# vghuy17ck1/svt-av1-psyex

Measured on AMD Instinct MI355X. Metric: ME+RD-cost Mpixels/s (2160p10 preset-6), higher is better.
Workload: dtype u8 SAD / i32 transforms; 1 GPU; 3840x2160 10-bit synthetic pan sequence, preset 6 (M6) search controls at qp 35; step = 16 pictures (4 current pictures x ref distance 1,2,4,8; R=2): open-loop ME of all 2040 b64 + full-pel pred + RD chain (64x64,32x32,16x16 DCT_DCT, 10-bit, b quantizer; qcoeff + recon + scalars written); 3 picture sets alternate from step to step

## Files before the change

svt-av1-psyex_amd/csrc/rd_kernel.hip:

```cpp
#include <hip/hip_runtime.h>
#include <math.h>
#include <stdint.h>
#include <string.h>
#include <type_traits>
#include "svt_hip_internal.h"
#include "../../include/svt_hip_dsp.h"

#include "txfm_core.h"

namespace {

struct RdParams {
    SvtHipRdBatchDesc d;
    const int16_t    *iscan[3];
    int               tx_size;
};

template <typename T> __device__ __forceinline__ int ldpix(const void *p, size_t i) { return (int)static_cast<const T *>(p)[i]; }

__host__ __device__ constexpr int rd_lanes_per_block(int ts) { return tx_wide(ts) > tx_high(ts) ? tx_wide(ts) : tx_high(ts); }
__host__ __device__ constexpr int rd_blocks_per_wave(int ts) { return 64 / rd_lanes_per_block(ts); }

#ifndef SVT_RD_WAVES_64
#define SVT_RD_WAVES_64 2
#endif
#ifndef SVT_RD_WAVES_32
#define SVT_RD_WAVES_32 4
#endif
#ifndef SVT_RD_RESIDUAL_AHEAD
#define SVT_RD_RESIDUAL_AHEAD 8
#endif
#ifndef SVT_RD_SCAN_AHEAD
#define SVT_RD_SCAN_AHEAD 16
#endif
#ifndef SVT_RD_WAVES_16
#define SVT_RD_WAVES_16 4
#endif
__host__ __device__ constexpr int rd_waves_per_simd(int ts) {
    return rd_lanes_per_block(ts) == 64 ? SVT_RD_WAVES_64 : rd_lanes_per_block(ts) == 32 ? SVT_RD_WAVES_32 : SVT_RD_WAVES_16;
}
template <int TS, int BD> __global__ void __launch_bounds__(64, rd_waves_per_simd(TS)) rd_tx_kernel(const RdParams p) {
    constexpr int W = tx_wide(TS), H = tx_high(TS), WP = W > 32 ? 32 : W, HP = H > 32 ? 32 : H, NP = WP * HP;
    constexpr int LW = rd_lanes_per_block(TS), BPW = rd_blocks_per_wave(TS);
    constexpr bool kShift32 = LW != 32;
    constexpr int PA = W + 1, PB = WP + 1;
    constexpr int ROW_CLAMP = BD == 8 ? 16 : 18, COL_CLAMP = 16;
    constexpr bool RECT = (W == 2 * H || H == 2 * W);
    using Pix = typename std::conditional<BD == 8, uint8_t, uint16_t>::type;
    __shared__ int32_t lds[BPW][H * PA];
    const int      lane = threadIdx.x, blk = lane / LW, l = lane % LW;
    const uint32_t job   = blockIdx.x * BPW + blk;
    const bool     valid = job < p.d.n_jobs;
    int32_t *A = lds[blk];
    const SvtHipTxJob jb = p.d.jobs[valid ? job : 0];
    const int tt = jb.tx_type & 15, vt = c_vtx[tt], ht = c_htx[tt];
    const bool ud = (vt == 2), lr = (ht == 2);
    const Pix *src  = static_cast<const Pix *>(p.d.src) + jb.src_offset;
    const Pix *pred = static_cast<const Pix *>(p.d.pred) + jb.pred_offset;
    const int8_t *fsh = c_fwd_shift[TS];
    const int bit_col = c_fwd_cos_col[ilog2c(W) - 2][ilog2c(H) - 2], bit_row = c_fwd_cos_row[ilog2c(W) - 2][ilog2c(H) - 2];

    constexpr int RUN = W < 8 ? W : 8, RPR = W / RUN;
    typedef Pix __attribute__((ext_vector_type(RUN), aligned(sizeof(Pix)))) RunU;
    uint32_t rmax = 0;
    {
        HiLo rhl;
        constexpr int NIT = (RPR * H + LW - 1) / LW, kResidualAhead = NIT < SVT_RD_RESIDUAL_AHEAD ? NIT : SVT_RD_RESIDUAL_AHEAD;
        for (int it0 = 0; it0 < NIT; it0 += kResidualAhead) {
            RunU sv[kResidualAhead], pv[kResidualAhead];
#pragma unroll
            for (int j = 0; j < kResidualAhead; j++) {
                const int i = l + (it0 + j) * LW;
                if (it0 + j < NIT && i < RPR * H) {
                    const int r = i / RPR, c = (i - r * RPR) * RUN;
                    sv[j] = *reinterpret_cast<const RunU *>(src + (size_t)r * p.d.src_stride + c);
                    pv[j] = *reinterpret_cast<const RunU *>(pred + (size_t)r * p.d.pred_stride + c);
                }
            }
#pragma unroll
            for (int j = 0; j < kResidualAhead; j++) {
                const int i = l + (it0 + j) * LW;
                if (it0 + j < NIT && i < RPR * H) {
                    const int r = i / RPR, c = (i - r * RPR) * RUN;
#pragma unroll
                    for (int k = 0; k < RUN; k++) {
                        const int32_t d = (int16_t)((int16_t)sv[j][k] - (int16_t)pv[j][k]);
                        A[r * PA + c + k] = d;
                        rhl.take(d);
                    }
                }
            }
        }
        rmax = rhl.max_abs();
    }
    const bool fast_col = pass_fits_17_bits((uint32_t)__builtin_amdgcn_readfirstlane((int)wave_max(rmax)) << (fsh[0] > 0 ? fsh[0] : 0), H);
    __syncthreads();
    uint32_t cmax = 0;
    if (l < W) {
        int32_t x[H];
#pragma unroll
        for (int r = 0; r < H; r++) x[r] = A[(ud ? H - 1 - r : r) * PA + l];
        shift_vec<H>(x, fsh[0]);
        if (fast_col) { fwd_1d<H, 2>(x, vt, bit_col); shift_vec<H, kShift32>(x, fsh[1]); } else { fwd_1d<H, 0>(x, vt, bit_col); shift_vec<H>(x, fsh[1]); }
        const int oc = lr ? W - 1 - l : l;
#pragma unroll
        for (int r = 0; r < H; r++) A[r * PA + oc] = x[r];
        cmax = vec_max_abs<H>(x);
    }
    const bool fast_row = pass_fits_17_bits((uint32_t)__builtin_amdgcn_readfirstlane((int)wave_max(cmax)), W);
    __syncthreads();
    uint32_t comax = 0;
    if (l < H) {
        int32_t x[W];
#pragma unroll
        for (int c = 0; c < W; c++) x[c] = A[l * PA + c];
        if (fast_row) { fwd_1d<W, 2>(x, ht, bit_row); shift_vec<W, kShift32>(x, fsh[2]); } else { fwd_1d<W, 0>(x, ht, bit_row); shift_vec<W>(x, fsh[2]); }
        if constexpr (RECT) {
#pragma unroll
            for (int c = 0; c < W; c++) x[c] = rshift64((i64)x[c] * 5793, 12);
        }
#pragma unroll
        for (int c = 0; c < W; c++) A[l * PA + c] = x[c];
        comax = vec_max_abs<W>(x);
    }
    const uint32_t comax_w = (uint32_t)__builtin_amdgcn_readfirstlane((int)wave_max(comax));
    const bool q24 = comax_w < (1u << 16);
    __syncthreads();
    const int pf = jb.pf_shape & 3;
    const int keep_w = pf == 3 ? 1 : (W >> pf), keep_h = pf == 3 ? 1 : (H >> pf);
    u64 tq = 0;
    if (pf == 0) if constexpr (W > 32 || H > 32) {
        for (int i = l; i < W * H; i += LW) {
            const int r = i / W, c = i - r * W;
            if (r >= HP || c >= WP) { const int32_t v = A[r * PA + c]; tq += (u64)((i64)v * v); }
        }
        tq = group_sum<LW>(tq);
    }
    if constexpr (W > 32 || H > 32) __syncthreads();
    const SvtHipQuantRow q = p.d.quant_rows[jb.quant_row];
    const int     log_scale = p.d.quant_kind == 2 ? 0 : c_log_scale[TS];
    const int16_t *iscan    = p.iscan[(tt >= 10) ? ((tt & 1) ? 2 : 1) : 0];
    const uint8_t *qm = (tt < 9) ? p.d.qmatrix : nullptr, *iqm = (tt < 9) ? p.d.iqmatrix : nullptr;
    uint32_t satd = 0, eob = 0, qsum = 0;
    int32_t  dc_q = 0;
    u64      dres = 0, dpred = 0;
    int32_t *co_out = (p.d.coeff && valid) ? p.d.coeff + (size_t)job * NP : nullptr;
    int32_t *q_out  = (p.d.qcoeff && valid) ? p.d.qcoeff + (size_t)job * NP : nullptr;
    int32_t *dq_out = (p.d.dqcoeff && valid) ? p.d.dqcoeff + (size_t)job * NP : nullptr;
    const int32_t zb_c[2]  = {log_scale ? ((q.zbin[0] + (1 << (log_scale - 1))) >> log_scale) : q.zbin[0], log_scale ? ((q.zbin[1] + (1 << (log_scale - 1))) >> log_scale) : q.zbin[1]};
    const int32_t rnd_c[2] = {log_scale ? ((q.round[0] + (1 << (log_scale - 1))) >> log_scale) : q.round[0], log_scale ? ((q.round[1] + (1 << (log_scale - 1))) >> log_scale) : q.round[1]};
    const bool fast_q = q24 && !qm && p.d.quant_kind == 0 && !co_out && !dq_out && __all(pf == 0);
    constexpr int LS = tx_log_scale(TS), KT = LS == 2 ? 4 : 3;
    bool lane_lean = fast_q && q_out != nullptr && log_scale == LS;
    {
        const int32_t  rndm = rnd_c[0] > rnd_c[1] ? rnd_c[0] : rnd_c[1], sm = q.quant_shift[0] > q.quant_shift[1] ? q.quant_shift[0] : q.quant_shift[1];
        const int32_t  dm = q.dequant[0] > q.dequant[1] ? q.dequant[0] : q.dequant[1], qm2 = (q.quant[0] > q.quant[1] ? q.quant[0] : q.quant[1]) + 65536;
        const bool     nonneg = (rnd_c[0] | rnd_c[1] | q.quant_shift[0] | q.quant_shift[1] | q.dequant[0] | q.dequant[1]) >= 0;
        uint32_t       tmax = comax_w + (uint32_t)(nonneg ? rndm : 0);
        if (BD == 8) tmax = tmax > 32767u ? 32767u : tmax;
        const u64 qvmax = ((((u64)tmax * (uint32_t)qm2) >> 11) * (u64)(uint32_t)(nonneg ? sm : 0)) >> (21 - LS);
        const u64 dqmax = (qvmax * (u64)(uint32_t)(nonneg ? dm : 0)) >> LS;
        const u64 M = dqmax > comax_w ? dqmax : (u64)comax_w;
        lane_lean = lane_lean && nonneg && tmax < (1u << (18 - KT)) && M < (1u << 16) && M * M * (NP / LW) < (1ull << 32);
    }
    const bool lean_q = __all(lane_lean);
    if (lean_q) {
        static_assert(NP % LW == 0, "every lane of a block walks the same number of coefficients");
        constexpr int kScanAhead = NP / LW < SVT_RD_SCAN_AHEAD ? ((NP / LW) & ~1) : SVT_RD_SCAN_AHEAD;
        static_assert(kScanAhead >= 2 && kScanAhead % 2 == 0 && NP / LW >= kScanAhead, "ahead of the loop");
// ... 137 lines not shown
                qv = (int32_t)(((((t * q.quant[ac]) >> 16) + t) * q.quant_shift[ac]) >> (16 - log_scale + 5));
                const int32_t deq = ((int32_t)q.dequant[ac] * iwt + 16) >> 5;
                dq = (qv * deq) >> log_scale;
            }
        } else if (!qm) {
            const bool keep = (BD == 8) ? (((i64)a << (1 + log_scale)) >= (int32_t)q.dequant[ac]) : ((a << (1 + log_scale)) >= q.dequant[ac]);
            if (keep) {
                i64 t = (i64)a + (log_scale ? ((q.round_fp[ac] + (1 << (log_scale - 1))) >> log_scale) : q.round_fp[ac]);
                if (BD == 8) t = t < -32768 ? -32768 : (t > 32767 ? 32767 : t);
                qv = (int32_t)((t * q.quant_fp[ac]) >> (16 - log_scale));
                dq = (qv * (int32_t)q.dequant[ac]) >> log_scale;
            }
        } else {
            if ((i64)a * wt >= ((int32_t)q.dequant[ac] << (5 - (1 + log_scale)))) {
                i64 t = (i64)a + (log_scale ? ((q.round_fp[ac] + (1 << (log_scale - 1))) >> log_scale) : q.round_fp[ac]);
                if (BD == 8) t = t < -32768 ? -32768 : (t > 32767 ? 32767 : t);
                qv = (int32_t)((t * q.quant_fp[ac] * wt) >> (16 - log_scale + 5));
                const int32_t deq = ((int32_t)q.dequant[ac] * iwt + 16) >> 5;
                dq = (qv * deq) >> log_scale;
            }
        }
        const int32_t qs = (qv ^ sign) - sign, dqs = (dq ^ sign) - sign;
        if (qv) { const uint32_t e = (uint32_t)iscan[rc] + 1; eob = e > eob ? e : eob; }
        qsum += (uint32_t)(qv > 63 ? 63 : qv);
        if (rc == 0) dc_q = qs;
        const i64 dd = (i64)co - dqs;
        dres += (u64)(dd * dd);
        dpred += (u64)((i64)co * co);
        A[r * PB + c] = dqs;
        if (co_out) co_out[rc] = co;
        if (q_out) q_out[rc] = qs;
        if (dq_out) dq_out[rc] = dqs;
    }
    satd  = group_sum<LW>(satd);
    qsum  = group_sum<LW>(qsum);
    eob   = group_max<LW>(eob);
    dres  = group_sum<LW>(dres);
    dpred = group_sum<LW>(dpred);
    __syncthreads();
    int32_t xr[W];
    uint32_t irmax = 0;
    if (l < H) {
#pragma unroll
        for (int c = 0; c < W; c++) {
            int32_t v = (l < HP && c < WP) ? A[l * PB + c] : 0;
            if constexpr (RECT) v = rshift64((i64)v * 2896, 12);
            xr[c] = clampv(v, BD + 8);
        }
        irmax = vec_max_abs<W>(xr);
    }
    const bool fast_irow = ipass_fits_18_bits((uint32_t)__builtin_amdgcn_readfirstlane((int)wave_max(irmax)), W);
    uint32_t icmax = 0;
    if (l < H) {
        if (fast_irow) inv_1d<W, ROW_CLAMP, 2>(xr, ht); else inv_1d<W, ROW_CLAMP, 1>(xr, ht);
        shift_vec<W, kShift32>(xr, c_inv_shift0[TS]);
#pragma unroll
        for (int c = 0; c < W; c++) A[l * PA + c] = xr[c];
        icmax = vec_max_abs<W>(xr);
    }
    const bool fast_icol = ipass_fits_18_bits((uint32_t)__builtin_amdgcn_readfirstlane((int)wave_max(icmax)), H);
    __syncthreads();
    u64 sse = 0;
    if (l < W) {
        int32_t x[H];
        const int ic = lr ? W - 1 - l : l;
#pragma unroll
        for (int r = 0; r < H; r++) x[r] = (r < HP) ? clampv(A[r * PA + ic], BD + 6 > 16 ? BD + 6 : 16) : 0;
        if (fast_icol) inv_1d<H, COL_CLAMP, 2>(x, vt); else inv_1d<H, COL_CLAMP, 1>(x, vt);
        shift_vec<H, kShift32>(x, -4);
#pragma unroll
        for (int r = 0; r < H; r++) A[r * PA + l] = x[ud ? H - 1 - r : r];
    }
    __syncthreads();
    {
        Pix *rec = (p.d.recon && valid) ? static_cast<Pix *>(p.d.recon) + jb.pred_offset : nullptr;
        constexpr int NIT = (RPR * H + LW - 1) / LW;
        RunU pv[NIT], sv[NIT];
#pragma unroll
        for (int it = 0; it < NIT; it++) {
            const int i = l + it * LW;
            if (i < RPR * H) {
                const int r = i / RPR, c = (i - r * RPR) * RUN;
                pv[it] = *reinterpret_cast<const RunU *>(pred + (size_t)r * p.d.pred_stride + c);
                sv[it] = *reinterpret_cast<const RunU *>(src + (size_t)r * p.d.src_stride + c);
            }
        }
#pragma unroll
        for (int it = 0; it < NIT; it++) {
            const int i = l + it * LW;
            if (i < RPR * H) {
                const int r = i / RPR, c = (i - r * RPR) * RUN;
                RunU out;
#pragma unroll
                for (int k = 0; k < RUN; k++) {
                    int v = (int)pv[it][k] + A[r * PA + c + k];
                    v = v < 0 ? 0 : (v > (1 << BD) - 1 ? (1 << BD) - 1 : v);
                    out[k] = (Pix)v;
                    const int e = (int)sv[it][k] - v;
                    sse += (u64)((uint32_t)e * (uint32_t)e);
                }
                if (rec) *reinterpret_cast<RunU *>(rec + (size_t)r * p.d.pred_stride + c) = out;
            }
        }
    }
    sse = group_sum<LW>(sse);
    if (l == 0 && valid) {
        p.d.eob[job]  = (uint16_t)eob;
        p.d.satd[job] = satd;
        p.d.dist_coeff[2 * (size_t)job]     = dres;
        p.d.dist_coeff[2 * (size_t)job + 1] = dpred;
        p.d.three_quad_energy[job] = tq;
        p.d.sse[job]  = sse;
        if (p.d.cul_level) p.d.cul_level[job] = (uint8_t)((qsum > 63 ? 63 : qsum) | (dc_q < 0 ? 64 : 0)) + (uint8_t)(dc_q > 0 ? 128 : 0);
    }
}

struct InvParams {
    SvtHipInvTxBatchDesc d;
};
template <int TS, int BD, typename Pix> __global__ void __launch_bounds__(64, rd_waves_per_simd(TS)) inv_tx_kernel(const InvParams p) {
    constexpr int W = tx_wide(TS), H = tx_high(TS), WP = W > 32 ? 32 : W, HP = H > 32 ? 32 : H, NP = WP * HP;
    constexpr int LW = rd_lanes_per_block(TS), BPW = rd_blocks_per_wave(TS);
    constexpr bool kShift32 = LW != 32;
    constexpr int PA = W + 1, PB = WP + 1;
    constexpr int ROW_CLAMP = BD == 8 ? 16 : 18, COL_CLAMP = 16;
    constexpr bool RECT = (W == 2 * H || H == 2 * W);
    __shared__ int32_t lds[BPW][H * PA];
    const int      lane = threadIdx.x, blk = lane / LW, l = lane % LW;
    const uint32_t job   = blockIdx.x * BPW + blk;
    const bool     valid = job < p.d.n_jobs;
    int32_t *A = lds[blk];
    const SvtHipTxJob jb = p.d.jobs[valid ? job : 0];
    const int tt = jb.tx_type & 15, vt = c_vtx[tt], ht = c_htx[tt];
    const bool ud = (vt == 2), lr = (ht == 2);
    const Pix *pred = static_cast<const Pix *>(p.d.pred) + jb.pred_offset;
    const int32_t *dq = p.d.dqcoeff + (size_t)(valid ? job : 0) * NP;
    for (int rc = l; rc < NP; rc += LW) { const int r = rc / WP, c = rc - r * WP; A[r * PB + c] = dq[rc]; }
    __syncthreads();
    int32_t xr[W];
    uint32_t irmax = 0;
    if (l < H) {
#pragma unroll
        for (int c = 0; c < W; c++) {
            int32_t v = (l < HP && c < WP) ? A[l * PB + c] : 0;
            if constexpr (RECT) v = rshift64((i64)v * 2896, 12);
            xr[c] = clampv(v, BD + 8);
        }
        irmax = vec_max_abs<W>(xr);
    }
    const bool fast_irow = ipass_fits_18_bits((uint32_t)__builtin_amdgcn_readfirstlane((int)wave_max(irmax)), W);
    uint32_t icmax = 0;
    if (l < H) {
        if (fast_irow) inv_1d<W, ROW_CLAMP, 2>(xr, ht); else inv_1d<W, ROW_CLAMP, 1>(xr, ht);
        shift_vec<W, kShift32>(xr, c_inv_shift0[TS]);
#pragma unroll
        for (int c = 0; c < W; c++) A[l * PA + c] = xr[c];
        icmax = vec_max_abs<W>(xr);
    }
    const bool fast_icol = ipass_fits_18_bits((uint32_t)__builtin_amdgcn_readfirstlane((int)wave_max(icmax)), H);
    __syncthreads();
    if (l < W) {
        int32_t x[H];
        const int ic = lr ? W - 1 - l : l;
#pragma unroll
        for (int r = 0; r < H; r++) x[r] = (r < HP) ? clampv(A[r * PA + ic], BD + 6 > 16 ? BD + 6 : 16) : 0;
        if (fast_icol) inv_1d<H, COL_CLAMP, 2>(x, vt); else inv_1d<H, COL_CLAMP, 1>(x, vt);
        shift_vec<H, kShift32>(x, -4);
#pragma unroll
        for (int r = 0; r < H; r++) A[r * PA + l] = x[ud ? H - 1 - r : r];
    }
    __syncthreads();
    if (valid) {
        Pix *rec = static_cast<Pix *>(p.d.recon) + jb.src_offset;
        for (int i = l; i < W * H; i += LW) {
            const int r = i / W, c = i - r * W;
            int v = (int)pred[(size_t)r * p.d.pred_stride + c] + A[r * PA + c];
            v = v < 0 ? 0 : (v > (1 << BD) - 1 ? (1 << BD) - 1 : v);
            rec[(size_t)r * p.d.recon_stride + c] = (Pix)v;
        }
    }
}

template <int BD, typename Pix> int launch_inv(SvtHipContext *ctx, const InvParams &p) {
    const dim3 b(64);
#define CASE(S) case S: hipLaunchKernelGGL((inv_tx_kernel<S, BD, Pix>), dim3((p.d.n_jobs + rd_blocks_per_wave(S) - 1) / rd_blocks_per_wave(S)), b, 0, ctx->stream, p); break;
    switch (p.d.tx_size) {
        CASE(0) CASE(1) CASE(2) CASE(3) CASE(4) CASE(5) CASE(6) CASE(7) CASE(8) CASE(9) CASE(10) CASE(11) CASE(12) CASE(13) CASE(14) CASE(15) CASE(16) CASE(17) CASE(18)
    default: return svt_hip_fail(ctx, SVT_HIP_ERR_BAD_PARAM, "tx_size %d", p.d.tx_size);
    }
#undef CASE
    SVT_HIP_CHECK(ctx, hipGetLastError());
    return SVT_HIP_OK;
}

struct FwdParams {
    SvtHipFwdTxBatchDesc d;
};
template <int TS> __global__ void __launch_bounds__(64, rd_waves_per_simd(TS)) fwd_tx_kernel(const FwdParams p) {
    constexpr int W = tx_wide(TS), H = tx_high(TS);
    constexpr int LW = rd_lanes_per_block(TS), BPW = rd_blocks_per_wave(TS);
    constexpr int PA = W + 1;
    constexpr bool RECT = (W == 2 * H || H == 2 * W);
    __shared__ int32_t lds[BPW][H * PA];
    const int      lane = threadIdx.x, blk = lane / LW, l = lane % LW;
    const uint32_t job   = blockIdx.x * BPW + blk;
    const bool     valid = job < p.d.n_jobs;
    int32_t *A = lds[blk];
    const SvtHipTxJob jb = p.d.jobs[valid ? job : 0];
    const int tt = jb.tx_type & 15, vt = c_vtx[tt], ht = c_htx[tt];
    const bool ud = (vt == 2), lr = (ht == 2);
    const int16_t *res = p.d.residual + jb.src_offset;
    const int8_t *fsh = c_fwd_shift[TS];
    const int bit_col = c_fwd_cos_col[ilog2c(W) - 2][ilog2c(H) - 2], bit_row = c_fwd_cos_row[ilog2c(W) - 2][ilog2c(H) - 2];
    uint32_t rmax = 0;
    for (int i = l; i < W * H; i += LW) {
        const int r = i / W, c = i - r * W;
        const int32_t d = res[(size_t)r * p.d.residual_stride + c];
        A[r * PA + c] = d;
        rmax = max(rmax, (uint32_t)(d < 0 ? -d : d));
    }
// ... 251 lines not shown
```

svt-av1-psyex_amd/csrc/txfm_core.h:

```cpp
#ifndef SVT_HIP_TXFM_CORE_H
#define SVT_HIP_TXFM_CORE_H
#include <hip/hip_runtime.h>
#include <math.h>
#include <stdint.h>
#include "wave_ops.h"

namespace {

typedef unsigned long long u64;
typedef long long          i64;

__constant__ int32_t c_cospi[4][64];
inline hipError_t txfm_upload_cospi() {
    int32_t cosp[4][64];
    for (int b = 0; b < 4; b++)
        for (int j = 0; j < 64; j++) cosp[b][j] = (int32_t)(cos(3.14159265358979323846 * j / 128.0) * (double)(1 << (10 + b)) + 0.5);
    return hipMemcpyToSymbol(HIP_SYMBOL(c_cospi), cosp, sizeof(cosp));
}
__constant__ int32_t c_sinpi[4][5] = {{0, 330, 621, 836, 951}, {0, 660, 1241, 1672, 1901}, {0, 1321, 2482, 3344, 3803}, {0, 2642, 4964, 6689, 7606}};

struct TxGeom { uint8_t w, h; };
__host__ __device__ constexpr int tx_wide(int s) { constexpr uint8_t t[19] = {4, 8, 16, 32, 64, 4, 8, 8, 16, 16, 32, 32, 64, 4, 16, 8, 32, 16, 64}; return t[s]; }
__host__ __device__ constexpr int tx_high(int s) { constexpr uint8_t t[19] = {4, 8, 16, 32, 64, 8, 4, 16, 8, 32, 16, 64, 32, 16, 4, 32, 8, 64, 16}; return t[s]; }
__host__ __device__ constexpr int ilog2c(int n) { return n <= 1 ? 0 : 1 + ilog2c(n >> 1); }
__host__ __device__ constexpr int brevc(int v, int bits) { int r = 0; for (int i = 0; i < bits; i++) r |= ((v >> i) & 1) << (bits - 1 - i); return r; }

__device__ const int8_t  c_fwd_shift[19][3] = {{2, 0, 0},  {2, -1, 0}, {2, -2, 0}, {2, -4, 0}, {0, -2, -2}, {2, -1, 0}, {2, -1, 0}, {2, -2, 0}, {2, -2, 0}, {2, -4, 0},
                                               {2, -4, 0}, {0, -2, -2}, {2, -4, -2}, {2, -1, 0}, {2, -1, 0}, {2, -2, 0}, {2, -2, 0}, {0, -2, 0}, {2, -4, 0}};
__device__ const int8_t  c_fwd_cos_col[5][5] = {{13, 13, 13, 0, 0}, {13, 13, 13, 12, 0}, {13, 13, 13, 12, 13}, {0, 13, 13, 12, 13}, {0, 0, 13, 12, 13}};
__device__ const int8_t  c_fwd_cos_row[5][5] = {{13, 13, 12, 0, 0}, {13, 13, 13, 12, 0}, {13, 13, 12, 13, 12}, {0, 12, 13, 12, 11}, {0, 0, 12, 11, 10}};
__device__ const int8_t  c_inv_shift0[19]    = {0, -1, -2, -2, -2, 0, 0, -1, -1, -1, -1, -1, -1, -1, -1, -2, -2, -2, -2};
__device__ const uint8_t c_log_scale[19]     = {0, 0, 0, 1, 2, 0, 0, 0, 0, 1, 1, 2, 2, 0, 0, 0, 0, 1, 1};
__device__ const uint8_t c_vtx[16] = {0, 1, 0, 1, 2, 0, 2, 1, 2, 3, 0, 3, 1, 3, 2, 3};
__device__ const uint8_t c_htx[16] = {0, 0, 1, 1, 0, 2, 2, 2, 1, 3, 3, 0, 3, 1, 3, 2};

__device__ __forceinline__ int32_t mul24_shr(int32_t a, int32_t b, int sh) {
    int32_t hi;
    asm("v_mul_hi_i32_i24 %0, %1, %2" : "=v"(hi) : "v"(a), "v"(b));
    return (int32_t)__builtin_amdgcn_alignbit((uint32_t)hi, (uint32_t)__mul24(a, b), (uint32_t)sh);
}
__device__ __forceinline__ uint32_t umul24_lo(uint32_t a, uint32_t b) {
    uint32_t lo;
    asm("v_mul_u32_u24 %0, %1, %2" : "=v"(lo) : "v"(a), "v"(b));
    return lo;
}
__device__ __forceinline__ uint32_t umul24_hi(uint32_t a, uint32_t b) {
    uint32_t hi;
    asm("v_mul_hi_u32_u24 %0, %1, %2" : "=v"(hi) : "v"(a), "v"(b));
    return hi;
}
__host__ __device__ constexpr int tx_log_scale(int s) { return tx_wide(s) * tx_high(s) > 1024 ? 2 : tx_wide(s) * tx_high(s) > 256 ? 1 : 0; }
__device__ __forceinline__ int32_t rshift64(i64 v, int bit) { return (int32_t)((v + ((i64)1 << (bit - 1))) >> bit); }
template <int MUL> __device__ __forceinline__ int32_t hbtf(int32_t w0, int32_t a, int32_t w1, int32_t b, int bit) {
    if constexpr (MUL == 2) return (__mul24(w1, b) + (__mul24(w0, a) + (1 << (bit - 1)))) >> bit;
    i64 s;
    if constexpr (MUL == 1) s = (i64)__mul24(w0, a) + (i64)__mul24(w1, b);
    else s = (i64)(int32_t)((uint32_t)w0 * (uint32_t)a) + (i64)(int32_t)((uint32_t)w1 * (uint32_t)b);
    return (int32_t)((s + ((i64)1 << (bit - 1))) >> bit);
}
__device__ __forceinline__ int32_t clamp32(int32_t v, int bit) {
    const int32_t hi = (1 << (bit - 1)) - 1, lo = -(1 << (bit - 1));
    return v < lo ? lo : (v > hi ? hi : v);
}
__device__ __forceinline__ int32_t clampv(i64 v, int bit) {
    const i64 hi = ((i64)1 << (bit - 1)) - 1, lo = -((i64)1 << (bit - 1));
    return (int32_t)(v < lo ? lo : (v > hi ? hi : v));
}
__device__ __forceinline__ int32_t clampv(int32_t v, int bit) { return clamp32(v, bit); }
__device__ __forceinline__ int32_t wadd(int32_t a, int32_t b) { return (int32_t)((uint32_t)a + (uint32_t)b); }
__device__ __forceinline__ int32_t wsub(int32_t a, int32_t b) { return (int32_t)((uint32_t)a - (uint32_t)b); }

template <int M, int K, int MUL> __device__ __forceinline__ void odd_rot(int32_t *x, const int32_t *c, int bit) {
    constexpr int t = M >> K;
    if constexpr (K == 1) {
#pragma unroll
        for (int j = 0; j < M / 4; j++) {
            const int p = M + M / 4 + j, m = 3 * M - 1 - p;
            const int32_t a = x[p], b = x[m];
            x[p] = hbtf<MUL>(-c[32], a, c[32], b, bit);
            x[m] = hbtf<MUL>(c[32], b, c[32], a, bit);
        }
    } else {
#pragma unroll
        for (int g = 0; g < (1 << (K - 2)); g++) {
            const int A = (1 + 4 * brevc(g, K - 2)) * (64 >> K), B = 64 - A, base = M + g * 2 * t;
#pragma unroll
            for (int j = 0; j < t / 2; j++) {
                const int p = base + t / 2 + j, m = 3 * M - 1 - p;
                const int32_t a = x[p], b = x[m];
                x[p] = hbtf<MUL>(-c[A], a, c[B], b, bit);
                x[m] = hbtf<MUL>(c[A], b, c[B], a, bit);
            }
#pragma unroll
            for (int j = 0; j < t / 2; j++) {
                const int p = base + t + j, m = 3 * M - 1 - p;
                const int32_t a = x[p], b = x[m];
                x[p] = hbtf<MUL>(-c[B], a, -c[A], b, bit);
                x[m] = hbtf<MUL>(c[B], b, -c[A], a, bit);
            }
        }
    }
}
template <int M, int K, int CLAMP> __device__ __forceinline__ void odd_bfly(int32_t *x) {
    constexpr int t = M >> K;
#pragma unroll
    for (int g = 0; g < M / t; g++) {
#pragma unroll
        for (int j = 0; j < t / 2; j++) {
            const int i0 = M + g * t + j, i1 = M + g * t + t - 1 - j;
            const int32_t lo = x[i0], hi = x[i1];
            int32_t s, d;
            if constexpr (CLAMP < 0) { s = wadd(lo, hi); d = (g & 1) ? wsub(hi, lo) : wsub(lo, hi); }
            else { s = clamp32(lo + hi, CLAMP); d = clamp32((g & 1) ? hi - lo : lo - hi, CLAMP); }
            x[i0] = (g & 1) ? d : s;
            x[i1] = (g & 1) ? s : d;
        }
    }
}
template <int M, bool INV, int MUL = INV ? 1 : 0> __device__ __forceinline__ void odd_final(int32_t *x, const int32_t *c, int bit) {
#pragma unroll
    for (int i = 0; i < M / 2; i++) {
        const int A = 64 - (2 * brevc(i, ilog2c(M)) + 1) * (32 / M), B = 64 - A, p = M + i, m = 2 * M - 1 - i;
        const int32_t a = x[p], b = x[m];
        if constexpr (!INV) { x[p] = hbtf<MUL>(c[A], a, c[B], b, bit); x[m] = hbtf<MUL>(c[A], b, -c[B], a, bit); }
        else { x[p] = hbtf<MUL>(c[A], a, -c[B], b, bit); x[m] = hbtf<MUL>(c[B], a, c[A], b, bit); }
    }
}
template <int M, int K, int FM> struct OddFwd {
    static __device__ __forceinline__ void run(int32_t *x, const int32_t *c, int bit) {
        if constexpr (K < ilog2c(M)) {
            odd_rot<M, K, FM>(x, c, bit);
            odd_bfly<M, K, -1>(x);
            OddFwd<M, K + 1, FM>::run(x, c, bit);
        }
    }
};
template <int M, int K, int CLAMP, int IM> struct OddInv {
    static __device__ __forceinline__ void run(int32_t *x, const int32_t *c, int bit) {
        if constexpr (K >= 1) {
            odd_bfly<M, K, CLAMP>(x);
            odd_rot<M, K, IM>(x, c, bit);
            OddInv<M, K - 1, CLAMP, IM>::run(x, c, bit);
        }
    }
};
template <int N, int FM> __device__ __forceinline__ void fdct_core(int32_t *x, const int32_t *c, int bit) {
    if constexpr (N == 2) {
        const int32_t a = x[0], b = x[1];
        x[0] = hbtf<FM>(c[32], a, c[32], b, bit);
        x[1] = hbtf<FM>(-c[32], b, c[32], a, bit);
    } else {
        constexpr int M = N / 2;
#pragma unroll
        for (int i = 0; i < M; i++) { const int32_t a = x[i], b = x[N - 1 - i]; x[i] = wadd(a, b); x[N - 1 - i] = wsub(a, b); }
        fdct_core<M, FM>(x, c, bit);
        OddFwd<M, 1, FM>::run(x, c, bit);
        odd_final<M, false, FM>(x, c, bit);
    }
}
template <int N, int CLAMP, int IM> __device__ __forceinline__ void idct_core(int32_t *x, const int32_t *c, int bit) {
    if constexpr (N == 2) {
        const int32_t a = x[0], b = x[1];
        x[0] = hbtf<IM>(c[32], a, c[32], b, bit);
        x[1] = hbtf<IM>(c[32], a, -c[32], b, bit);
    } else {
        constexpr int M = N / 2;
        odd_final<M, true, IM>(x, c, bit);
        OddInv<M, ilog2c(M) - 1, CLAMP, IM>::run(x, c, bit);
        idct_core<M, CLAMP, IM>(x, c, bit);
#pragma unroll
        for (int i = 0; i < M; i++) { const int32_t a = x[i], b = x[N - 1 - i]; x[i] = clamp32(a + b, CLAMP); x[N - 1 - i] = clamp32(a - b, CLAMP); }
    }
}
template <int N> __device__ __forceinline__ void permute_brev(int32_t *x) {
#pragma unroll
    for (int k = 0; k < N; k++) {
        const int r = brevc(k, ilog2c(N));
        if (r > k) { const int32_t t = x[k]; x[k] = x[r]; x[r] = t; }
    }
}

template <int N> __host__ __device__ constexpr int adst_perm(int k) {
    if constexpr (N == 2) return k;
    else return (k & 1) ? N - 1 - adst_perm<N / 2>(k >> 1) : adst_perm<N / 2>(k >> 1);
}
template <int N, int HH, int MUL> __device__ __forceinline__ void adst_rot(int32_t *x, const int32_t *c, int bit) {
#pragma unroll
    for (int b = 0; b < N; b += 2 * HH) {
        if constexpr (HH == 2) {
            const int32_t a = x[b + 2], d = x[b + 3];
            x[b + 2] = hbtf<MUL>(c[32], a, c[32], d, bit);
            x[b + 3] = hbtf<MUL>(c[32], a, -c[32], d, bit);
        } else {
#pragma unroll
            for (int j = 0; j < HH / 4; j++) {
                const int A = (4 * j + 1) * (64 / HH), B = 64 - A, p = b + HH + 2 * j, q = b + HH + HH / 2 + 2 * j;
                int32_t a = x[p], d = x[p + 1];
                x[p]     = hbtf<MUL>(c[A], a, c[B], d, bit);
                x[p + 1] = hbtf<MUL>(c[B], a, -c[A], d, bit);
                a = x[q]; d = x[q + 1];
                x[q]     = hbtf<MUL>(-c[B], a, c[A], d, bit);
                x[q + 1] = hbtf<MUL>(c[A], a, c[B], d, bit);
            }
        }
    }
}
template <int N, int HH, int CLAMP> __device__ __forceinline__ void adst_bfly(int32_t *x) {
#pragma unroll
    for (int b = 0; b < N; b += 2 * HH)
#pragma unroll
        for (int j = 0; j < HH; j++) {
            const int32_t a = x[b + j], d = x[b + j + HH];
            if constexpr (CLAMP < 0) { x[b + j] = wadd(a, d); x[b + j + HH] = wsub(a, d); }
            else { x[b + j] = clamp32(a + d, CLAMP); x[b + j + HH] = clamp32(a - d, CLAMP); }
        }
}
template <int N, int MUL> __device__ __forceinline__ void adst_last(int32_t *x, const int32_t *c, int bit) {
#pragma unroll
    for (int j = 0; j < N / 2; j++) {
        const int A = (4 * j + 1) * (64 / (2 * N)), B = 64 - A;
        const int32_t a = x[2 * j], d = x[2 * j + 1];
        x[2 * j]     = hbtf<MUL>(c[A], a, c[B], d, bit);
        x[2 * j + 1] = hbtf<MUL>(c[B], a, -c[A], d, bit);
    }
}
template <int N, int HH, int FM> struct AdstFwd {
    static __device__ __forceinline__ void run(int32_t *x, const int32_t *c, int bit) {
        if constexpr (HH < N) { adst_rot<N, HH, FM>(x, c, bit); adst_bfly<N, HH, -1>(x); AdstFwd<N, HH * 2, FM>::run(x, c, bit); }
    }
};
template <int N, int HH, int CLAMP, int IM> struct AdstInv {
    static __device__ __forceinline__ void run(int32_t *x, const int32_t *c, int bit) {
        if constexpr (HH >= 2) { adst_bfly<N, HH, CLAMP>(x); adst_rot<N, HH, IM>(x, c, bit); AdstInv<N, HH / 2, CLAMP, IM>::run(x, c, bit); }
    }
};
template <int N, int FM> __device__ __forceinline__ void fadst(int32_t *x, const int32_t *c, int bit) {
    int32_t y[N];
#pragma unroll
    for (int k = 0; k < N; k++) { const int32_t v = x[adst_perm<N>(k)]; y[k] = (__builtin_popcount(k) & 1) ? (int32_t)(0u - (uint32_t)v) : v; }
    AdstFwd<N, 2, FM>::run(y, c, bit);
    adst_last<N, FM>(y, c, bit);
#pragma unroll
    for (int j = 0; j < N / 2; j++) { x[2 * j] = y[2 * j + 1]; x[2 * j + 1] = y[N - 2 - 2 * j]; }
}
template <int N, int CLAMP, int IM> __device__ __forceinline__ void iadst(int32_t *x, const int32_t *c, int bit) {
    int32_t y[N];
#pragma unroll
    for (int j = 0; j < N / 2; j++) { y[2 * j + 1] = x[2 * j]; y[N - 2 - 2 * j] = x[2 * j + 1]; }
    adst_last<N, IM>(y, c, bit);
    AdstInv<N, N / 2, CLAMP, IM>::run(y, c, bit);
#pragma unroll
    for (int k = 0; k < N; k++) x[adst_perm<N>(k)] = (__builtin_popcount(k) & 1) ? (int32_t)(0u - (uint32_t)y[k]) : y[k];
}
#define MUL32(a, b) ((int32_t)((uint32_t)(a) * (uint32_t)(b)))
__device__ __forceinline__ void adst4(int32_t *x, int bit, bool inverse) {
    const int32_t *s = c_sinpi[bit - 10];
    const int32_t x0 = x[0], x1 = x[1], x2 = x[2], x3 = x[3];
    if (!(x0 | x1 | x2 | x3)) return;
    if (!inverse) {
        const int32_t s7 = wsub(wadd(x0, x1), x3);
        const int32_t a0 = wadd(wadd(MUL32(s[1], x0), MUL32(s[2], x1)), MUL32(s[4], x3)), a1 = MUL32(s[3], s7);
        const int32_t a2 = wadd(wsub(MUL32(s[4], x0), MUL32(s[1], x1)), MUL32(s[2], x3)), a3 = MUL32(s[3], x2);
        x[0] = rshift64(wadd(a0, a3), bit); x[1] = rshift64(a1, bit); x[2] = rshift64(wsub(a2, a3), bit); x[3] = rshift64(wadd(wsub(a2, a0), a3), bit);
    } else {
        const int32_t s7 = wadd(wsub(x0, x2), x3);
        const int32_t a0 = wadd(wadd(MUL32(s[1], x0), MUL32(s[4], x2)), MUL32(s[2], x3));
        const int32_t a1 = wsub(wsub(MUL32(s[2], x0), MUL32(s[1], x2)), MUL32(s[4], x3)), a3 = MUL32(s[3], x1), a2 = MUL32(s[3], s7);
        x[0] = rshift64(wadd(a0, a3), bit); x[1] = rshift64(wadd(a1, a3), bit); x[2] = rshift64(a2, bit); x[3] = rshift64(wsub(wadd(a0, a1), a3), bit);
    }
}
template <int N> __device__ __forceinline__ void identity(int32_t *x) {
#pragma unroll
    for (int i = 0; i < N; i++) {
        if constexpr (N == 4) x[i] = rshift64((i64)x[i] * 5793, 12);
        else if constexpr (N == 8) x[i] = (int32_t)((uint32_t)x[i] * 2u);
        else if constexpr (N == 16) x[i] = rshift64((i64)x[i] * 2 * 5793, 12);
        else if constexpr (N == 32) x[i] = (int32_t)((uint32_t)x[i] * 4u);
        else x[i] = rshift64((i64)x[i] * 4 * 5793, 12);
    }
}
template <int N, int FM> __device__ __forceinline__ void fwd_1d(int32_t *x, int type, int bit) {
    const int32_t *c = c_cospi[bit - 10];
    if (type == 3) identity<N>(x);
    else if (type == 0) { fdct_core<N, FM>(x, c, bit); permute_brev<N>(x); }
    else if constexpr (N == 4) adst4(x, bit, false);
    else if constexpr (N <= 16) fadst<N, FM>(x, c, bit);
}
__device__ __forceinline__ bool pass_fits_17_bits(uint32_t wave_max_abs_input, int n) { return (unsigned long long)wave_max_abs_input * (unsigned)n < (1u << 17); }
template <int N, int CLAMP, int IM> __device__ __forceinline__ void inv_1d(int32_t *x, int type) {
    const int32_t *c = c_cospi[2];
    if (type == 3) identity<N>(x);
    else if (type == 0) { permute_brev<N>(x); idct_core<N, CLAMP, IM>(x, c, 12); }
    else if constexpr (N == 4) adst4(x, 12, true);
    else if constexpr (N <= 16) iadst<N, CLAMP, IM>(x, c, 12);
}
__device__ __forceinline__ bool ipass_fits_18_bits(uint32_t wave_max_abs_input, int n) { return (unsigned long long)wave_max_abs_input * (unsigned)n < (1u << 18); }
struct HiLo {
    int32_t hi = 0, lo = 0;
    __device__ __forceinline__ void take(int32_t a, int32_t b) { hi = max(max(hi, a), b); lo = min(min(lo, a), b); }
    __device__ __forceinline__ void take(int32_t a) { hi = max(hi, a); lo = min(lo, a); }
    __device__ __forceinline__ uint32_t max_abs() const { return (uint32_t)max(hi, -lo); }
};
template <int N> __device__ __forceinline__ uint32_t vec_max_abs(const int32_t *x) {
    HiLo m;
    if constexpr (N % 2 == 0) {
#pragma unroll
        for (int i = 0; i < N; i += 2) m.take(x[i], x[i + 1]);
    } else {
#pragma unroll
        for (int i = 0; i < N; i++) m.take(x[i]);
    }
    return m.max_abs();
}
template <int N, bool SAFE32 = false> __device__ __forceinline__ void shift_vec(int32_t *x, int sh) {
    if (sh < 0) {
#pragma unroll
        for (int i = 0; i < N; i++) x[i] = SAFE32 ? ((x[i] + (1 << (-sh - 1))) >> -sh) : rshift64(x[i], -sh);
    } else if (sh > 0) {
#pragma unroll
        for (int i = 0; i < N; i++) x[i] = (int32_t)((uint32_t)x[i] << sh);
    }
}

}
#endif
```

Baseline: 42930 Mpixels/s.

## Fold post-transform shifts into butterfly rounding and use scalar-weight mad24 in bounded passes

Result: faster. 43970 Mpixels/s (median of 6 runs) (+2.4%).

```diff
diff --git a/svt-av1-psyex_amd/csrc/rd_kernel.hip b/svt-av1-psyex_amd/csrc/rd_kernel.hip
--- a/svt-av1-psyex_amd/csrc/rd_kernel.hip
+++ b/svt-av1-psyex_amd/csrc/rd_kernel.hip
@@ -36,6 +36,12 @@
 #ifndef SVT_RD_WAVES_16
 #define SVT_RD_WAVES_16 4
 #endif
+#ifndef SVT_RD_FOLD_INV_32LANE
+#define SVT_RD_FOLD_INV_32LANE 1
+#endif
+__host__ __device__ constexpr int rd_bounded_btf(int ts) {
+    return ((rd_lanes_per_block(ts) == 32 && tx_wide(ts) != tx_high(ts)) || (tx_wide(ts) == 64 && tx_high(ts) == 16)) ? 3 : 2;
+}
 __host__ __device__ constexpr int rd_waves_per_simd(int ts) {
     return rd_lanes_per_block(ts) == 64 ? SVT_RD_WAVES_64 : rd_lanes_per_block(ts) == 32 ? SVT_RD_WAVES_32 : SVT_RD_WAVES_16;
 }
@@ -43,6 +49,8 @@
     constexpr int W = tx_wide(TS), H = tx_high(TS), WP = W > 32 ? 32 : W, HP = H > 32 ? 32 : H, NP = WP * HP;
     constexpr int LW = rd_lanes_per_block(TS), BPW = rd_blocks_per_wave(TS);
     constexpr bool kShift32 = LW != 32;
+    constexpr bool kFoldInv = LW != 32 || SVT_RD_FOLD_INV_32LANE;
+    constexpr int kBtf = rd_bounded_btf(TS);
     constexpr int PA = W + 1, PB = WP + 1;
     constexpr int ROW_CLAMP = BD == 8 ? 16 : 18, COL_CLAMP = 16;
     constexpr bool RECT = (W == 2 * H || H == 2 * W);
@@ -101,7 +109,11 @@
 #pragma unroll
         for (int r = 0; r < H; r++) x[r] = A[(ud ? H - 1 - r : r) * PA + l];
         shift_vec<H>(x, fsh[0]);
-        if (fast_col) { fwd_1d<H, 2>(x, vt, bit_col); shift_vec<H, kShift32>(x, fsh[1]); } else { fwd_1d<H, 0>(x, vt, bit_col); shift_vec<H>(x, fsh[1]); }
+        if constexpr (kBtf == 2) {
+#pragma unroll
+            for (int r = 0; r < H; r++) x[r] = held_in_vgpr(x[r]);
+        }
+        if (fast_col) fwd_1d_bounded<H, kShift32, kBtf>(x, vt, bit_col, fsh[1]); else { fwd_1d<H, 0>(x, vt, bit_col); shift_vec<H>(x, fsh[1]); }
         const int oc = lr ? W - 1 - l : l;
 #pragma unroll
         for (int r = 0; r < H; r++) A[r * PA + oc] = x[r];
@@ -114,7 +126,7 @@
         int32_t x[W];
 #pragma unroll
         for (int c = 0; c < W; c++) x[c] = A[l * PA + c];
-        if (fast_row) { fwd_1d<W, 2>(x, ht, bit_row); shift_vec<W, kShift32>(x, fsh[2]); } else { fwd_1d<W, 0>(x, ht, bit_row); shift_vec<W>(x, fsh[2]); }
+        if (fast_row) fwd_1d_bounded<W, kShift32, kBtf>(x, ht, bit_row, fsh[2]); else { fwd_1d<W, 0>(x, ht, bit_row); shift_vec<W>(x, fsh[2]); }
         if constexpr (RECT) {
 #pragma unroll
             for (int c = 0; c < W; c++) x[c] = rshift64((i64)x[c] * 5793, 12);
@@ -358,8 +370,8 @@
     const bool fast_irow = ipass_fits_18_bits((uint32_t)__builtin_amdgcn_readfirstlane((int)wave_max(irmax)), W);
     uint32_t icmax = 0;
     if (l < H) {
-        if (fast_irow) inv_1d<W, ROW_CLAMP, 2>(xr, ht); else inv_1d<W, ROW_CLAMP, 1>(xr, ht);
-        shift_vec<W, kShift32>(xr, c_inv_shift0[TS]);
+        if (fast_irow) inv_1d_bounded<W, ROW_CLAMP, kShift32, kFoldInv, kBtf>(xr, ht, c_inv_shift0[TS]);
+        else { inv_1d<W, ROW_CLAMP, 1>(xr, ht); shift_vec<W, kShift32>(xr, c_inv_shift0[TS]); }
 #pragma unroll
         for (int c = 0; c < W; c++) A[l * PA + c] = xr[c];
         icmax = vec_max_abs<W>(xr);
@@ -372,8 +384,8 @@
         const int ic = lr ? W - 1 - l : l;
 #pragma unroll
         for (int r = 0; r < H; r++) x[r] = (r < HP) ? clampv(A[r * PA + ic], BD + 6 > 16 ? BD + 6 : 16) : 0;
-        if (fast_icol) inv_1d<H, COL_CLAMP, 2>(x, vt); else inv_1d<H, COL_CLAMP, 1>(x, vt);
-        shift_vec<H, kShift32>(x, -4);
+        if (fast_icol) inv_1d_bounded<H, COL_CLAMP, kShift32, kFoldInv, kBtf>(x, vt, -4);
+        else { inv_1d<H, COL_CLAMP, 1>(x, vt); shift_vec<H, kShift32>(x, -4); }
 #pragma unroll
         for (int r = 0; r < H; r++) A[r * PA + l] = x[ud ? H - 1 - r : r];
     }
@@ -427,7 +439,8 @@
 template <int TS, int BD, typename Pix> __global__ void __launch_bounds__(64, rd_waves_per_simd(TS)) inv_tx_kernel(const InvParams p) {
     constexpr int W = tx_wide(TS), H = tx_high(TS), WP = W > 32 ? 32 : W, HP = H > 32 ? 32 : H, NP = WP * HP;
     constexpr int LW = rd_lanes_per_block(TS), BPW = rd_blocks_per_wave(TS);
-    constexpr bool kShift32 = LW != 32;
+    constexpr bool kShift32 = LW != 32, kFoldInv = LW != 32 || SVT_RD_FOLD_INV_32LANE;
+    constexpr int kBtf = rd_bounded_btf(TS);
     constexpr int PA = W + 1, PB = WP + 1;
     constexpr int ROW_CLAMP = BD == 8 ? 16 : 18, COL_CLAMP = 16;
     constexpr bool RECT = (W == 2 * H || H == 2 * W);
@@ -457,8 +470,8 @@
     const bool fast_irow = ipass_fits_18_bits((uint32_t)__builtin_amdgcn_readfirstlane((int)wave_max(irmax)), W);
     uint32_t icmax = 0;
     if (l < H) {
-        if (fast_irow) inv_1d<W, ROW_CLAMP, 2>(xr, ht); else inv_1d<W, ROW_CLAMP, 1>(xr, ht);
-        shift_vec<W, kShift32>(xr, c_inv_shift0[TS]);
+        if (fast_irow) inv_1d_bounded<W, ROW_CLAMP, kShift32, kFoldInv, kBtf>(xr, ht, c_inv_shift0[TS]);
+        else { inv_1d<W, ROW_CLAMP, 1>(xr, ht); shift_vec<W, kShift32>(xr, c_inv_shift0[TS]); }
 #pragma unroll
         for (int c = 0; c < W; c++) A[l * PA + c] = xr[c];
         icmax = vec_max_abs<W>(xr);
@@ -470,8 +483,8 @@
         const int ic = lr ? W - 1 - l : l;
 #pragma unroll
         for (int r = 0; r < H; r++) x[r] = (r < HP) ? clampv(A[r * PA + ic], BD + 6 > 16 ? BD + 6 : 16) : 0;
-        if (fast_icol) inv_1d<H, COL_CLAMP, 2>(x, vt); else inv_1d<H, COL_CLAMP, 1>(x, vt);
-        shift_vec<H, kShift32>(x, -4);
+        if (fast_icol) inv_1d_bounded<H, COL_CLAMP, kShift32, kFoldInv, kBtf>(x, vt, -4);
+        else { inv_1d<H, COL_CLAMP, 1>(x, vt); shift_vec<H, kShift32>(x, -4); }
 #pragma unroll
         for (int r = 0; r < H; r++) A[r * PA + l] = x[ud ? H - 1 - r : r];
     }
diff --git a/svt-av1-psyex_amd/csrc/txfm_core.h b/svt-av1-psyex_amd/csrc/txfm_core.h
--- a/svt-av1-psyex_amd/csrc/txfm_core.h
+++ b/svt-av1-psyex_amd/csrc/txfm_core.h
@@ -51,13 +51,60 @@
 }
 __host__ __device__ constexpr int tx_log_scale(int s) { return tx_wide(s) * tx_high(s) > 1024 ? 2 : tx_wide(s) * tx_high(s) > 256 ? 1 : 0; }
 __device__ __forceinline__ int32_t rshift64(i64 v, int bit) { return (int32_t)((v + ((i64)1 << (bit - 1))) >> bit); }
-template <int MUL> __device__ __forceinline__ int32_t hbtf(int32_t w0, int32_t a, int32_t w1, int32_t b, int bit) {
-    if constexpr (MUL == 2) return (__mul24(w1, b) + (__mul24(w0, a) + (1 << (bit - 1)))) >> bit;
+#ifndef SVT_TX_FOLD_FWD
+#define SVT_TX_FOLD_FWD 1
+#endif
+#ifndef SVT_TX_FOLD_INV
+#define SVT_TX_FOLD_INV 1
+#endif
+struct Btf {
+    int     bit;
+    int32_t rnd;
+    int     obit;
+    int32_t ornd;
+};
+__device__ __forceinline__ int32_t held_in_vgpr(int32_t v) {
+    asm("" : "+v"(v));
+    return v;
+}
+__device__ __forceinline__ Btf btf_plain(int bit) { return Btf{bit, 0, bit, 0}; }
+__device__ __forceinline__ Btf btf_bounded(int bit) {
+    const int32_t r = held_in_vgpr(1 << (bit - 1));
+    return Btf{bit, r, bit, r};
+}
+__device__ __forceinline__ Btf btf_folded(int bit, int s) {
+    const int32_t r = held_in_vgpr(1 << (bit - 1));
+    if (s <= 0) return Btf{bit, r, bit, r};
+    return Btf{bit, r, bit + s, held_in_vgpr((1 << (bit - 1)) + (1 << (s - 1 + bit)))};
+}
+__device__ __forceinline__ int32_t mad24_sv(int32_t w, int32_t a, int32_t acc) {
+    int32_t r;
+    asm("v_mad_i32_i24 %0, %1, %2, %3" : "=v"(r) : "s"(w), "v"(a), "v"(acc));
+    return r;
+}
+__device__ __forceinline__ int32_t hbtf2(int32_t w0, int32_t a, int32_t w1, int32_t b, int32_t rnd, int bit) {
+    bool za = false, zb = false;
+    if (__builtin_constant_p(a) && a == 0) za = true;
+    if (__builtin_constant_p(b) && b == 0) zb = true;
+    if (za && zb) return 0;
+    int32_t acc = rnd;
+    if (!za) acc = mad24_sv(w0, a, acc);
+    if (!zb) acc = mad24_sv(w1, b, acc);
+    return acc >> bit;
+}
+template <int MUL> __device__ __forceinline__ int32_t hbtf(int32_t w0, int32_t a, int32_t w1, int32_t b, const Btf &P) {
+    if constexpr (MUL == 2) return hbtf2(w0, a, w1, b, P.rnd, P.bit);
+    const int bit = P.bit;
+    if constexpr (MUL == 3) return (__mul24(w1, b) + (__mul24(w0, a) + (1 << (bit - 1)))) >> bit;
     i64 s;
     if constexpr (MUL == 1) s = (i64)__mul24(w0, a) + (i64)__mul24(w1, b);
     else s = (i64)(int32_t)((uint32_t)w0 * (uint32_t)a) + (i64)(int32_t)((uint32_t)w1 * (uint32_t)b);
     return (int32_t)((s + ((i64)1 << (bit - 1))) >> bit);
 }
+template <int MUL> __device__ __forceinline__ int32_t hbtf_out(int32_t w0, int32_t a, int32_t w1, int32_t b, const Btf &P) {
+    if constexpr (MUL == 2) return hbtf2(w0, a, w1, b, P.ornd, P.obit);
+    else return hbtf<MUL>(w0, a, w1, b, P);
+}
 __device__ __forceinline__ int32_t clamp32(int32_t v, int bit) {
     const int32_t hi = (1 << (bit - 1)) - 1, lo = -(1 << (bit - 1));
     return v < lo ? lo : (v > hi ? hi : v);
@@ -70,7 +117,7 @@
 __device__ __forceinline__ int32_t wadd(int32_t a, int32_t b) { return (int32_t)((uint32_t)a + (uint32_t)b); }
 __device__ __forceinline__ int32_t wsub(int32_t a, int32_t b) { return (int32_t)((uint32_t)a - (uint32_t)b); }
 
-template <int M, int K, int MUL> __device__ __forceinline__ void odd_rot(int32_t *x, const int32_t *c, int bit) {
+template <int M, int K, int MUL> __device__ __forceinline__ void odd_rot(int32_t *x, const int32_t *c, const Btf &bit) {
     constexpr int t = M >> K;
     if constexpr (K == 1) {
 #pragma unroll
@@ -117,17 +164,17 @@
         }
     }
 }
-template <int M, bool INV, int MUL = INV ? 1 : 0> __device__ __forceinline__ void odd_final(int32_t *x, const int32_t *c, int bit) {
+template <int M, bool INV, int MUL = INV ? 1 : 0> __device__ __forceinline__ void odd_final(int32_t *x, const int32_t *c, const Btf &bit) {
 #pragma unroll
     for (int i = 0; i < M / 2; i++) {
         const int A = 64 - (2 * brevc(i, ilog2c(M)) + 1) * (32 / M), B = 64 - A, p = M + i, m = 2 * M - 1 - i;
         const int32_t a = x[p], b = x[m];
-        if constexpr (!INV) { x[p] = hbtf<MUL>(c[A], a, c[B], b, bit); x[m] = hbtf<MUL>(c[A], b, -c[B], a, bit); }
+        if constexpr (!INV) { x[p] = hbtf_out<MUL>(c[A], a, c[B], b, bit); x[m] = hbtf_out<MUL>(c[A], b, -c[B], a, bit); }
         else { x[p] = hbtf<MUL>(c[A], a, -c[B], b, bit); x[m] = hbtf<MUL>(c[B], a, c[A], b, bit); }
     }
 }
 template <int M, int K, int FM> struct OddFwd {
-    static __device__ __forceinline__ void run(int32_t *x, const int32_t *c, int bit) {
+    static __device__ __forceinline__ void run(int32_t *x, const int32_t *c, const Btf &bit) {
         if constexpr (K < ilog2c(M)) {
             odd_rot<M, K, FM>(x, c, bit);
             odd_bfly<M, K, -1>(x);
@@ -136,7 +183,7 @@
     }
 };
 template <int M, int K, int CLAMP, int IM> struct OddInv {
-    static __device__ __forceinline__ void run(int32_t *x, const int32_t *c, int bit) {
+    static __device__ __forceinline__ void run(int32_t *x, const int32_t *c, const Btf &bit) {
         if constexpr (K >= 1) {
             odd_bfly<M, K, CLAMP>(x);
             odd_rot<M, K, IM>(x, c, bit);
@@ -144,11 +191,11 @@
         }
     }
 };
-template <int N, int FM> __device__ __forceinline__ void fdct_core(int32_t *x, const int32_t *c, int bit) {
+template <int N, int FM> __device__ __forceinline__ void fdct_core(int32_t *x, const int32_t *c, const Btf &bit) {
     if constexpr (N == 2) {
         const int32_t a = x[0], b = x[1];
-        x[0] = hbtf<FM>(c[32], a, c[32], b, bit);
-        x[1] = hbtf<FM>(-c[32], b, c[32], a, bit);
+        x[0] = hbtf_out<FM>(c[32], a, c[32], b, bit);
+        x[1] = hbtf_out<FM>(-c[32], b, c[32], a, bit);
     } else {
         constexpr int M = N / 2;
 #pragma unroll
@@ -158,7 +205,7 @@
         odd_final<M, false, FM>(x, c, bit);
     }
 }
-template <int N, int CLAMP, int IM> __device__ __forceinline__ void idct_core(int32_t *x, const int32_t *c, int bit) {
+template <int N, int CLAMP, int IM> __device__ __forceinline__ void idct_core(int32_t *x, const int32_t *c, const Btf &bit, int out_s = 0) {
     if constexpr (N == 2) {
         const int32_t a = x[0], b = x[1];
         x[0] = hbtf<IM>(c[32], a, c[32], b, bit);
@@ -169,7 +216,14 @@
         OddInv<M, ilog2c(M) - 1, CLAMP, IM>::run(x, c, bit);
         idct_core<M, CLAMP, IM>(x, c, bit);
 #pragma unroll
-        for (int i = 0; i < M; i++) { const int32_t a = x[i], b = x[N - 1 - i]; x[i] = clamp32(a + b, CLAMP); x[N - 1 - i] = clamp32(a - b, CLAMP); }
+        for (int i = 0; i < M; i++) {
+            const int32_t a = x[i], b = x[N - 1 - i];
+            if (out_s > 0) {
+                const int32_t r = 1 << (out_s - 1), lo = -(1 << (CLAMP - 1)) + r, hi = (1 << (CLAMP - 1)) - 1 + r, t = a + r;
+                x[i]         = max(min(t + b, hi), lo) >> out_s;
+                x[N - 1 - i] = max(min(t - b, hi), lo) >> out_s;
+            } else { x[i] = clamp32(a + b, CLAMP); x[N - 1 - i] = clamp32(a - b, CLAMP); }
+        }
     }
 }
 template <int N> __device__ __forceinline__ void permute_brev(int32_t *x) {
@@ -184,7 +238,7 @@
     if constexpr (N == 2) return k;
     else return (k & 1) ? N - 1 - adst_perm<N / 2>(k >> 1) : adst_perm<N / 2>(k >> 1);
 }
-template <int N, int HH, int MUL> __device__ __forceinline__ void adst_rot(int32_t *x, const int32_t *c, int bit) {
+template <int N, int HH, int MUL> __device__ __forceinline__ void adst_rot(int32_t *x, const int32_t *c, const Btf &bit) {
 #pragma unroll
     for (int b = 0; b < N; b += 2 * HH) {
         if constexpr (HH == 2) {
@@ -215,39 +269,39 @@
             else { x[b + j] = clamp32(a + d, CLAMP); x[b + j + HH] = clamp32(a - d, CLAMP); }
         }
 }
-template <int N, int MUL> __device__ __forceinline__ void adst_last(int32_t *x, const int32_t *c, int bit) {
+template <int N, int MUL, bool OUT> __device__ __forceinline__ void adst_last(int32_t *x, const int32_t *c, const Btf &bit) {
 #pragma unroll
     for (int j = 0; j < N / 2; j++) {
         const int A = (4 * j + 1) * (64 / (2 * N)), B = 64 - A;
         const int32_t a = x[2 * j], d = x[2 * j + 1];
-        x[2 * j]     = hbtf<MUL>(c[A], a, c[B], d, bit);
-        x[2 * j + 1] = hbtf<MUL>(c[B], a, -c[A], d, bit);
+        if constexpr (OUT) { x[2 * j] = hbtf_out<MUL>(c[A], a, c[B], d, bit); x[2 * j + 1] = hbtf_out<MUL>(c[B], a, -c[A], d, bit); }
+        else { x[2 * j] = hbtf<MUL>(c[A], a, c[B], d, bit); x[2 * j + 1] = hbtf<MUL>(c[B], a, -c[A], d, bit); }
     }
 }
 template <int N, int HH, int FM> struct AdstFwd {
-    static __device__ __forceinline__ void run(int32_t *x, const int32_t *c, int bit) {
+    static __device__ __forceinline__ void run(int32_t *x, const int32_t *c, const Btf &bit) {
         if constexpr (HH < N) { adst_rot<N, HH, FM>(x, c, bit); adst_bfly<N, HH, -1>(x); AdstFwd<N, HH * 2, FM>::run(x, c, bit); }
     }
 };
 template <int N, int HH, int CLAMP, int IM> struct AdstInv {
-    static __device__ __forceinline__ void run(int32_t *x, const int32_t *c, int bit) {
+    static __device__ __forceinline__ void run(int32_t *x, const int32_t *c, const Btf &bit) {
         if constexpr (HH >= 2) { adst_bfly<N, HH, CLAMP>(x); adst_rot<N, HH, IM>(x, c, bit); AdstInv<N, HH / 2, CLAMP, IM>::run(x, c, bit); }
     }
 };
-template <int N, int FM> __device__ __forceinline__ void fadst(int32_t *x, const int32_t *c, int bit) {
+template <int N, int FM> __device__ __forceinline__ void fadst(int32_t *x, const int32_t *c, const Btf &bit) {
     int32_t y[N];
 #pragma unroll
     for (int k = 0; k < N; k++) { const int32_t v = x[adst_perm<N>(k)]; y[k] = (__builtin_popcount(k) & 1) ? (int32_t)(0u - (uint32_t)v) : v; }
     AdstFwd<N, 2, FM>::run(y, c, bit);
-    adst_last<N, FM>(y, c, bit);
+    adst_last<N, FM, true>(y, c, bit);
 #pragma unroll
     for (int j = 0; j < N / 2; j++) { x[2 * j] = y[2 * j + 1]; x[2 * j + 1] = y[N - 2 - 2 * j]; }
 }
-template <int N, int CLAMP, int IM> __device__ __forceinline__ void iadst(int32_t *x, const int32_t *c, int bit) {
+template <int N, int CLAMP, int IM> __device__ __forceinline__ void iadst(int32_t *x, const int32_t *c, const Btf &bit) {
     int32_t y[N];
 #pragma unroll
     for (int j = 0; j < N / 2; j++) { y[2 * j + 1] = x[2 * j]; y[N - 2 - 2 * j] = x[2 * j + 1]; }
-    adst_last<N, IM>(y, c, bit);
+    adst_last<N, IM, false>(y, c, bit);
     AdstInv<N, N / 2, CLAMP, IM>::run(y, c, bit);
 #pragma unroll
     for (int k = 0; k < N; k++) x[adst_perm<N>(k)] = (__builtin_popcount(k) & 1) ? (int32_t)(0u - (uint32_t)y[k]) : y[k];
@@ -281,18 +335,20 @@
 }
 template <int N, int FM> __device__ __forceinline__ void fwd_1d(int32_t *x, int type, int bit) {
     const int32_t *c = c_cospi[bit - 10];
+    const Btf P = FM == 2 ? btf_bounded(bit) : btf_plain(bit);
     if (type == 3) identity<N>(x);
-    else if (type == 0) { fdct_core<N, FM>(x, c, bit); permute_brev<N>(x); }
+    else if (type == 0) { fdct_core<N, FM>(x, c, P); permute_brev<N>(x); }
     else if constexpr (N == 4) adst4(x, bit, false);
-    else if constexpr (N <= 16) fadst<N, FM>(x, c, bit);
+    else if constexpr (N <= 16) fadst<N, FM>(x, c, P);
 }
 __device__ __forceinline__ bool pass_fits_17_bits(uint32_t wave_max_abs_input, int n) { return (unsigned long long)wave_max_abs_input * (unsigned)n < (1u << 17); }
 template <int N, int CLAMP, int IM> __device__ __forceinline__ void inv_1d(int32_t *x, int type) {
     const int32_t *c = c_cospi[2];
+    const Btf P = IM == 2 ? btf_bounded(12) : btf_plain(12);
     if (type == 3) identity<N>(x);
-    else if (type == 0) { permute_brev<N>(x); idct_core<N, CLAMP, IM>(x, c, 12); }
+    else if (type == 0) { permute_brev<N>(x); idct_core<N, CLAMP, IM>(x, c, P); }
     else if constexpr (N == 4) adst4(x, 12, true);
-    else if constexpr (N <= 16) iadst<N, CLAMP, IM>(x, c, 12);
+    else if constexpr (N <= 16) iadst<N, CLAMP, IM>(x, c, P);
 }
 __device__ __forceinline__ bool ipass_fits_18_bits(uint32_t wave_max_abs_input, int n) { return (unsigned long long)wave_max_abs_input * (unsigned)n < (1u << 18); }
 struct HiLo {
@@ -322,5 +378,42 @@
     }
 }
 
-}
+template <int N, bool SAFE32, int BM = 2> __device__ __forceinline__ void fwd_1d_bounded(int32_t *x, int type, int bit, int sh) {
+    if constexpr (BM != 2) {
+        fwd_1d<N, BM>(x, type, bit);
+        shift_vec<N, SAFE32>(x, sh);
+        return;
+    }
+#if SVT_TX_FOLD_FWD
+    const int32_t *c = c_cospi[bit - 10];
+    const Btf P = btf_folded(bit, -sh);
+    if (type == 3) { identity<N>(x); shift_vec<N, SAFE32>(x, sh); }
+    else if (type == 0) { fdct_core<N, 2>(x, c, P); permute_brev<N>(x); }
+    else if constexpr (N == 4) { adst4(x, bit, false); shift_vec<N, SAFE32>(x, sh); }
+    else if constexpr (N <= 16) fadst<N, 2>(x, c, P);
+#else
+    fwd_1d<N, 2>(x, type, bit);
+    shift_vec<N, SAFE32>(x, sh);
 #endif
+}
+template <int N, int CLAMP, bool SAFE32, bool FOLD, int BM = 2> __device__ __forceinline__ void inv_1d_bounded(int32_t *x, int type, int sh) {
+    const int32_t *c = c_cospi[2];
+    if constexpr (BM != 2) {
+        inv_1d<N, CLAMP, BM>(x, type);
+        shift_vec<N, SAFE32>(x, sh);
+        return;
+    }
+    if (type == 3) { identity<N>(x); shift_vec<N, SAFE32>(x, sh); }
+    else if (type == 0) {
+        permute_brev<N>(x);
+        if constexpr (FOLD && SVT_TX_FOLD_INV && (CLAMP > 16 || !SAFE32)) idct_core<N, CLAMP, 2>(x, c, btf_bounded(12), -sh);
+        else { idct_core<N, CLAMP, 2>(x, c, btf_bounded(12)); shift_vec<N, SAFE32>(x, sh); }
+    } else {
+        if constexpr (N == 4) adst4(x, 12, true);
+        else if constexpr (N <= 16) iadst<N, CLAMP, 2>(x, c, btf_bounded(12));
+        shift_vec<N, SAFE32>(x, sh);
+    }
+}
+
+}
+#endif
```
